# google/tfp-causalimpact

Hardware: AMD Instinct MI355X
Metric: posterior samples/sec (T=1000, 10 covariates) (higher is better)
Workload: dtype f32; 1 GPU; cfg2: T=1000, 10 covariates (P=11), LocalLinearTrend + spike-and-slab regression, Gibbs, W=112, S=1000; sampler=gibbs, chains_per_gpu=8, chains_total=8, parallelism=chains sharded over 1 GPU(s), no data-path collective, launcher=single process, collectives=none, ranks_seen=1

## Files before the change

tfp-causalimpact_amd/csrc/ci_api.hip:

```cpp
#include <hip/hip_runtime.h>

#include <algorithm>
#include <cerrno>
#include <cmath>
#include <cstdarg>
#include <cstdio>
#include <cstring>
#include <mutex>
#include <string>
#include <tuple>
#include <vector>

#include "../../include/causalimpact_amd.h"
#include "ci_kernels.h"
#include "ci_kernels8.h"
#define CI_SEASONAL_DECL_ONLY
#include "ci_seasonal.h"
#include "ci_wide.h"
#include "ci_seasonal_tp.h"
#include "ci_summary.h"
#include "ci_hmc.h"
#include "ci_score_seq.h"
#include "ci_gibbs64.h"
#include "ci_wide_score.h"
// ... 553 lines not shown
  if (pb->T < 3) return fail("T must be >= 3, got %d", pb->T);
  if (pb->P < 0 || pb->P > ci::MAXP_BIG)
    return fail("P must be in [0, %d], got %d", ci::MAXP_BIG, pb->P);
  if (pb->num_blocks < 0 || pb->num_blocks > CI_MAX_BLOCKS)
    return fail("num_blocks must be in [0, %d], got %d", CI_MAX_BLOCKS, pb->num_blocks);
  if (pb->num_blocks > 0) {
    int dfull = pb->has_slope ? 2 : 1;
    for (int k = 0; k < pb->num_blocks; ++k) {
      if (pb->num_seasons[k] < 2) return fail("num_seasons[%d] must be >= 2", k);
      dfull += pb->num_seasons[k];
    }
    if (use_wide(pb)) {
      if (wide_steps_per_thread(pb->T) > ci::WIDE_MAX_LC)
        return fail("T=%d exceeds the time-parallel seasonal path (max %d)", pb->T, ci::NT * ci::WIDE_MAX_LC);
    } else {
      if (dfull > ci::MW_MAXD)
        return fail("seasonal state too wide: %d > %d components (the limit of the multi-wavefront "
                    "seasonal kernel)", dfull, ci::MW_MAXD);
    }
  }
  if (pb->num_warmup < 0 || pb->num_results < 1) return fail("need num_warmup >= 0, num_results >= 1");
  if (pb->num_chains < 1 || pb->num_series < 1) return fail("need num_chains >= 1, num_series >= 1");
  if (pb->series_offset < 0 || pb->chain_offset < 0) return fail("series_offset and chain_offset must be >= 0");
  if (pb->num_blocks == 0 && steps_per_thread(pb->T) == 0 &&
      wide_steps_per_thread(pb->T) > ci::WIDE_MAX_LC)
    return fail("T=%d exceeds the longest supported series (%d)", pb->T, ci::NT * ci::WIDE_MAX_LC);
  return 0;
}

int ci_session_destroy(ci_session* s);

struct SessionGuard {
  ci_session* s;
  ~SessionGuard() { if (s) ci_session_destroy(s); }
};

static int validate_ragged(const ci_problem* pb, const int32_t* series_lengths) {
  if (validate(pb)) return 1;
  if (!series_lengths) return fail("series_lengths is NULL");
  if (pb->num_blocks > 0)
    return fail("ragged sessions hold trend models only: num_blocks must be 0, got %d", pb->num_blocks);
  if (pb->P > ci::MAXP)
    return fail("ragged sessions take at most %d design columns, got P=%d", ci::MAXP, pb->P);
  const int L = steps_per_thread(pb->T);
  if (L == 0)
    return fail("ragged sessions take series of at most %d steps, got T=%d", ci::NT * 16, pb->T);
  int longest = 0;
  for (int b = 0; b < pb->num_series; ++b) {
    const int tb = series_lengths[b];
    if (tb < 3) return fail("series_lengths[%d] must be >= 3, got %d", b, tb);
    if (tb > pb->T) return fail("series_lengths[%d] = %d exceeds the stride T=%d", b, tb, pb->T);
    if (tb > longest) longest = tb;
  }
  if (longest != pb->T)
    return fail("T must be the longest series of the session: max(series_lengths) = %d, T = %d",
                longest, pb->T);
  for (int b = 0; b < pb->num_series; ++b)
    if (steps_per_thread(series_lengths[b]) != L)
      return fail("series_lengths[%d] = %d runs %d steps per thread, the longest series (%d) runs %d: "
                  "all series of a ragged session must share that class",
                  b, series_lengths[b], steps_per_thread(series_lengths[b]), pb->T, L);
  return 0;
}

static int session_create_impl(const ci_problem* pb, const int32_t* series_lengths,
                               const int32_t* series_ids, const float* y, const uint8_t* mask,
                               const float* X, const uint8_t* season_change,
                               const ci_series_params* params, ci_session** out);

int ci_session_create(const ci_problem* pb, const float* y, const uint8_t* mask, const float* X,
                      const uint8_t* season_change, const ci_series_params* params,
                      ci_session** out) {
  if (validate(pb)) return 1;
  return session_create_impl(pb, nullptr, nullptr, y, mask, X, season_change, params, out);
}

int ci_session_create_ragged(const ci_problem* pb, const int32_t* series_lengths,
                             const int32_t* series_ids, const float* y, const uint8_t* mask,
                             const float* X, const ci_series_params* params, ci_session** out) {
  if (validate_ragged(pb, series_lengths)) return 1;
  if (series_ids)
    for (int b = 0; b < pb->num_series; ++b)
      if (series_ids[b] < 0) return fail("series_ids[%d] must be >= 0, got %d", b, series_ids[b]);
  return session_create_impl(pb, series_lengths, series_ids, y, mask, X, nullptr, params, out);
}

static int session_create_impl(const ci_problem* pb, const int32_t* series_lengths,
                               const int32_t* series_ids, const float* y, const uint8_t* mask,
                               const float* X, const uint8_t* season_change,
                               const ci_series_params* params, ci_session** out) {
  const bool ragged = series_lengths != nullptr;
  if (!y || !mask || !params || !out) return fail("NULL argument");
  if (pb->num_blocks > 0 && !season_change) return fail("season_change is NULL but num_blocks > 0");
  if (pb->P > 0 && !X) return fail("X is NULL but P=%d", pb->P);
  HIP_TRY(hipSetDevice(pb->device));
  ci_session* s = new ci_session();
  SessionGuard guard{s};
  s->pb = *pb;
  s->ragged = ragged;
  if (ragged) s->lengths.assign(series_lengths, series_lengths + pb->num_series);
  const ci_problem* caller_pb = pb;
  s->kpb = *pb;
  const bool bigp = pb->P > ci::MAXP;
  const bool long_trend = pb->num_blocks == 0 && ((steps_per_thread(pb->T) == 0 && !bigp) || wide_bigp_ok(pb));
  std::vector<uint8_t> no_changes;
  if (long_trend) {
    s->kpb.num_blocks = 1;
    s->kpb.num_seasons[0] = 2;
    s->kpb.flags &= ~CI_FLAG_SEQUENTIAL_SEASONAL;
    no_changes.assign((size_t)pb->T, 0);
    season_change = no_changes.data();
  }
  pb = &s->kpb;
  const int T = pb->T, P = pb->P, B = pb->num_series, C = pb->num_chains, S = pb->num_results;
  const int D = pb->has_slope ? 2 : 1;
  const int K = pb->num_blocks;
  (void)caller_pb;
  if (K == 0 && !bigp) {
    s->L = steps_per_thread(T);
    const ci::LdsLayout with_x = ci::make_layout(P, D, ci::NT * s->L, 1);
    s->x_in_lds = (P > 0 && with_x.total <= 150 * 1024) ? 1 : 0;
    s->lds_bytes = ci::make_layout(P, D, ci::NT * s->L, s->x_in_lds).total;
    const int pm = (P == 0) ? 0 : (P <= 16 ? (s->x_in_lds ? 1 : 3) : 2);
    s->fn = ragged ? pick_ragged_kernel(D, s->L, pm) : pick_kernel(D, s->L, pm);
    s->fn_prof = ragged ? nullptr : pick_kernel(D, s->L, pm + 8);
    if (!s->fn || (!ragged && !s->fn_prof)) return fail("no kernel for L=%d", s->L);
    char nm[96];
    snprintf(nm, sizeof(nm), ragged ? "ci::gibbs_kernel<%d,%d,%d,false,ragged>" : "ci::gibbs_kernel<%d,%d,%d,false>",
             D, s->L, pm);
    s->kernel_name = nm;
    int num_cus = 256;
    (void)hipDeviceGetAttribute(&num_cus, hipDeviceAttributeMultiprocessorCount, pb->device);
    const bool latency_regime = (long long)B * C <= (long long)num_cus;
    if ((pm == 1 || pm == 3) && latency_regime && !(pb->flags & CI_FLAG_FOUR_WAVES) && !ragged) {
      size_t base8 = 0;
      KernelFn f8 = pick_kernel8(D, s->L, 0, 0, &base8);
      size_t lds8 = base8 + (size_t)P * ci::NT * s->L * sizeof(float);
      int xg = 0;
      if (!f8 || lds8 > 160 * 1024) {
        f8 = pick_kernel8(D, s->L, 0, 1, &base8);
        lds8 = base8;
        xg = 1;
      }
      if (f8 && lds8 <= 160 * 1024) {
        s->fn = f8;
        s->fn_prof8 = xg ? nullptr : pick_kernel8(D, s->L, 1, 0, nullptr);
        if (s->fn_prof8)
          HIP_TRY(hipFuncSetAttribute((const void*)s->fn_prof8,
                                      hipFuncAttributeMaxDynamicSharedMemorySize, (int)lds8));
        s->eight_waves = true;
        if (const char* e_ = getenv("CI_SCHED_WORD")) {
          char* end_ = nullptr;
          const long v_ = strtol(e_, &end_, 0);
          if (end_ == e_ || *end_ != 0 || v_ < 0 || v_ > 0xFFFF)
            return fail("CI_SCHED_WORD must be an integer in [0, 65535], got '%s'", e_);
          s->sched_word = (int)v_;
        }
        s->lds_bytes = lds8;
        snprintf(nm, sizeof(nm), xg ? "ci::gibbs_kernel8<%d,%d,L2>" : "ci::gibbs_kernel8<%d,%d>", D, s->L);
        s->kernel_name = nm;
      }
    }
  } else {
    s->D_full = D;
    s->dred = D;
    for (int k = 0; k < K; ++k) { s->D_full += pb->num_seasons[k]; s->dred += pb->num_seasons[k] - 1; }
    s->wide = use_wide(pb);
    if (s->wide) {
      s->Lc = ci::wide_quad_steps(T);
      s->lds_bytes = ci::make_wlayout(P, s->dred).total;
      s->fn = (KernelFn)(bigp ? pick_wide_bigp_kernel(pb->has_slope, pb->num_seasons[0])
                              : pick_wide_kernel(pb->has_slope, pb->num_seasons[0]));
    } else {
      s->mw = s->D_full > 64 || (pb->flags & CI_FLAG_MULTIWAVE_SEASONAL) != 0;
      const int nwv = s->mw ? ci::MW_NWV : 1;
      const ci::SLayout in_lds = ci::make_slayout(T, P, K, s->D_full, s->dred, pb->has_slope, 0, nwv);
      s->seasonal_gws = in_lds.total > 150 * 1024 || (pb->flags & CI_FLAG_SEASONAL_WORKSPACE) != 0;
      const ci::SLayout lay = ci::make_slayout(T, P, K, s->D_full, s->dred, pb->has_slope,
                                               s->seasonal_gws ? 1 : 0, nwv);
      s->lds_bytes = lay.total;
      s->seasonal_ws_bytes = ((lay.t_total + 255) & ~(size_t)255) + (bigp ? ci::bigp_workspace_bytes(P) : 0);
    }
    const int tp_min_t = P > ci::MAXP ? 64 : 112;
    if (!s->wide && !s->mw && s->D_full <= ci::TP_MAXD && T >= tp_min_t && !(pb->flags & CI_FLAG_SEQUENTIAL_SEASONAL) &&
        !(pb->flags & CI_FLAG_SEASONAL_WORKSPACE)) {
      int num_cus = 256;
      (void)hipDeviceGetAttribute(&num_cus, hipDeviceAttributeMultiprocessorCount, pb->device);
      const long long groups = ((long long)B * C + 7) / 8 * 8;
      const ci::TpLds tl = ci::make_tplds(P, s->D_full);
      if (tl.total <= 160 * 1024) {
        int G = 1;
        while (G < ci::TP_MAXG && T / (2 * G * ci::TP_NWV) >= 16) G *= 2;
        int Gc = 1;
        if (!(pb->flags & CI_FLAG_NO_CLUSTER))
          while (Gc < G && groups * (2 * Gc) <= num_cus) Gc *= 2;
        s->tp = true;
        s->cluster = Gc;
        s->Lc = G;
        s->lds_bytes = tl.total;
        s->tp_ws_bytes = ci::make_tplayout(T, P, K, s->D_full, pb->has_slope, G).total;
        const int nq = ci::tp_nr(s->D_full) / 4;
        typedef void* (*TpFn)(void);
        static const TpFn tp_fns[9] = {nullptr, nullptr, ci_gibbs_seasonal_tp_fn_nq2, ci_gibbs_seasonal_tp_fn_nq3,
                                       ci_gibbs_seasonal_tp_fn_nq4, ci_gibbs_seasonal_tp_fn_nq5,
                                       ci_gibbs_seasonal_tp_fn_nq6, ci_gibbs_seasonal_tp_fn_nq7,
                                       ci_gibbs_seasonal_tp_fn_nq8};
        s->fn = (KernelFn)tp_fns[nq]();
      }
    }
    if (s->lds_bytes > 160 * 1024) {
      return fail("seasonal model needs %zu bytes of LDS per chain (max 163840): fewer covariates "
                  "or a narrower seasonal state", s->lds_bytes);
    }
    if (!s->wide && !s->tp) {
      const int which = (s->seasonal_gws ? 1 : 0) | (bigp ? 2 : 0);
      s->fn = (KernelFn)(s->mw ? ci_gibbs_seasonal_mw_fn(which) : ci_gibbs_seasonal_fn(which));
    }
    char nm[96];
    if (s->tp) snprintf(nm, sizeof(nm), "ci::gibbs_seasonal_tp_kernel<%d> %d chunks x%d", ci::tp_nr(s->D_full) / 4,
                        s->Lc * ci::TP_NWV, s->cluster);
    else if (s->wide) snprintf(nm, sizeof(nm), bigp ? "ci::gibbs_wide_kernel<%d,%d,bigp>" : "ci::gibbs_wide_kernel<%d,%d>", D, pb->num_seasons[0]);
    else if (s->mw) snprintf(nm, sizeof(nm), "ci::gibbs_seasonal_kernel<%s,%s,%d> (multi-wave)",
                             s->seasonal_gws ? "true" : "false", bigp ? "true" : "false", ci::MW_NWV);
    else snprintf(nm, sizeof(nm), "ci::gibbs_seasonal_kernel<%s,%s>", s->seasonal_gws ? "true" : "false",
                  bigp ? "true" : "false");
    s->kernel_name = nm;
  }
  HIP_TRY(hipFuncSetAttribute((const void*)s->fn, hipFuncAttributeMaxDynamicSharedMemorySize,
                              (int)s->lds_bytes));
  if (s->fn_prof) {
    const size_t lds_prof = K == 0 ? ci::make_layout(P, D, ci::NT * s->L, s->x_in_lds).total : s->lds_bytes;
    HIP_TRY(hipFuncSetAttribute((const void*)s->fn_prof, hipFuncAttributeMaxDynamicSharedMemorySize,
                                (int)lds_prof));
  }
  HIP_TRY(pool_stream_get(&s->stream));
  HIP_TRY(pool_event_get(&s->ev0));
  HIP_TRY(pool_event_get(&s->ev1));

  const size_t BT = (size_t)B * T, BCS = (size_t)B * C * S;
  HIP_TRY(s->y.alloc(BT));
  HIP_TRY(s->mask.alloc(BT));
  HIP_TRY(s->Xt.alloc((size_t)B * P * T));
  HIP_TRY(s->xtx.alloc((size_t)B * P * P));
  HIP_TRY(s->omega.alloc((size_t)B * P * P));
  HIP_TRY(s->wps.alloc(B));
  HIP_TRY(s->sp.alloc(B));
  HIP_TRY(s->o_obs.alloc(BCS));
  HIP_TRY(s->o_lscale.alloc(BCS));
  HIP_TRY(s->o_sscale.alloc(BCS));
  HIP_TRY(s->o_w.alloc(BCS * P));
  HIP_TRY(s->o_level.alloc(BCS * T));
  HIP_TRY(s->o_slope.alloc(pb->has_slope ? BCS * T : 0));
  HIP_TRY(s->o_pm.alloc((size_t)B * C * T));
  HIP_TRY(s->o_traj.alloc(BCS * T));
  if (ragged) {
    HIP_TRY(hipMemset(s->o_level.p, 0, s->o_level.n * sizeof(float)));
    if (s->o_slope.n) HIP_TRY(hipMemset(s->o_slope.p, 0, s->o_slope.n * sizeof(float)));
    HIP_TRY(hipMemset(s->o_pm.p, 0, s->o_pm.n * sizeof(float)));
    HIP_TRY(hipMemset(s->o_traj.p, 0, s->o_traj.n * sizeof(float)));
    HIP_TRY(s->series_T.alloc(B));
    HIP_TRY(hipMemcpy(s->series_T.p, series_lengths, B * sizeof(int), hipMemcpyHostToDevice));
    if (series_ids) {
      HIP_TRY(s->series_ids.alloc(B));
      HIP_TRY(hipMemcpy(s->series_ids.p, series_ids, B * sizeof(int), hipMemcpyHostToDevice));
    }
  }
  if (K > 0 || bigp) {
    HIP_TRY(s->season_change.alloc((size_t)K * T));
    HIP_TRY(s->ssp.alloc(B));
    HIP_TRY(s->p1_chol.alloc((size_t)B * s->dred * s->dred));
    s->inert_block = long_trend;
    if (!long_trend) {
      HIP_TRY(s->o_drift.alloc(BCS * K));
      HIP_TRY(s->o_seasonal.alloc(BCS * T * K));
    }
    if (s->wide) {
      HIP_TRY(s->ws.alloc((size_t)B * C * ci::wide_workspace_floats(s->dred, s->Lc)));
      int num_cus = 256;
      (void)hipDeviceGetAttribute(&num_cus, hipDeviceAttributeMultiprocessorCount, pb->device);
      const long long groups = ((long long)B * C + 7) / 8 * 8;
      s->cluster = 1;
      if (!(pb->flags & CI_FLAG_NO_CLUSTER) && P > 0 && (T & 3) == 0) {
        if (groups * 16 <= num_cus) s->cluster = 16;
        else if (groups * 8 <= num_cus) s->cluster = 8;
        else if (groups * 4 <= num_cus) s->cluster = 4;
        else if (groups * 2 <= num_cus) s->cluster = 2;
      }
      if ((s->cluster == 16 || s->cluster == 8) && getenv("CI_WIDE_DK_GLOBAL") == nullptr) {
        const size_t need = ci::make_wlayout(P, s->dred).big0 + ci::wide_dk_lds_bytes(s->Lc);
        if (need <= 160 * 1024 - 256) {
          s->dk_lds = 1;
          if (need > s->lds_bytes) {
            s->lds_bytes = need;
            HIP_TRY(hipFuncSetAttribute((const void*)s->fn, hipFuncAttributeMaxDynamicSharedMemorySize,
                                        (int)s->lds_bytes));
          }
        }
      }
      const size_t nseg = ((size_t)(T >> 2) + ci::NT - 1) / ci::NT;
      const size_t RS = (size_t)(P > 16 ? P : 16) + 4;
      HIP_TRY(s->csync.alloc((size_t)B * C * ci::CL_INTS));
      HIP_TRY(s->cpart.alloc((size_t)B * C * (nseg > 0 ? nseg : 1) * ci::NW * RS));
      HIP_TRY(s->cw.alloc((size_t)B * C * ci::wide_cw_floats(P)));
      HIP_TRY(s->cv.alloc((size_t)B * C * ci::wide_cv_doubles(P)));
    }
    else if (s->tp) {
      HIP_TRY(s->ws.alloc((size_t)B * C * (s->tp_ws_bytes / sizeof(float))));
      HIP_TRY(s->csync.alloc((size_t)B * C * ci::TPC_INTS));
// ... 1372 lines not shown
```

tfp-causalimpact_amd/csrc/ci_kernels8.h:

```cpp
#pragma once
#include "ci_kernels.h"

namespace ci {

constexpr int SCHED_DEFAULT = (2 << 4) | (1 << 6) | (0 << 8) | (2 << 10) | (2 << 12) | (0 << 14);
constexpr int NT8 = 512;
constexpr int NW8 = 8;
constexpr int PRE_MAXS = 16;

struct PreTables {
  double* tsw;
  double* V;
  double* rdk;
  double* hand;
};
constexpr size_t PRE_HALF_DOUBLES = PRE_MAXS * 16 + 16 * 16 + 16;
__host__ __device__ constexpr size_t pre_tables_bytes() {
  return sizeof(double) * (2 * PRE_HALF_DOUBLES + 20) + 16;
}
__device__ __forceinline__ PreTables pre_tables_at(unsigned char* base, int parity) {
  PreTables tb;
  double* d = (double*)base + (size_t)(parity & 1) * PRE_HALF_DOUBLES;
  tb.tsw = d; d += PRE_MAXS * 16;
  tb.V = d; d += 16 * 16;
  tb.rdk = d;
  tb.hand = (double*)base + 2 * PRE_HALF_DOUBLES;
  return tb;
}
constexpr int HAND_SCALE = 16, HAND_INTS = 17;

struct PreState {
  double c[4];
  double diag;
  double rdk;
  unsigned long long S;
  int n_sw;
  int valid;
};

template <int CTRL> __device__ __forceinline__ double dpp_ror_add_d(double v) {
  const int lo = __builtin_amdgcn_update_dpp(0, __double2loint(v), CTRL, 0xF, 0xF, false);
  const int hi = __builtin_amdgcn_update_dpp(0, __double2hiint(v), CTRL, 0xF, 0xF, false);
  return v + __hiloint2double(hi, lo);
}
__device__ __forceinline__ double row_sum16_d(double v) {
  v = dpp_ror_add_d<0x128>(v);
  v = dpp_ror_add_d<0x124>(v);
  v = dpp_ror_add_d<0x122>(v);
  v = dpp_ror_add_d<0x121>(v);
  return readlane_d(v, 0);
}

template <int KR>
__device__ __forceinline__ void sweep_rec_kr(QCols& m, int k, int lane, double& t_out, double& rd_out) {
  const int kq = k >> 2, j = lane & 15, q = lane >> 4;
  const double ckr = m.c[KR];
  const double rd = fast_rcp(readlane_d(ckr, k + 16 * kq));
  const double rowk = bperm_d(ckr, j + 16 * kq);
  const bool isk = j == k;
  const double t = isk ? 1.0 : rowk * rd;
  double colk[4];
#pragma unroll
  for (int r = 0; r < 4; ++r) colk[r] = bperm_d(m.c[r], k + 16 * q);
  __builtin_amdgcn_sched_barrier(0);
#pragma unroll
  for (int r = 0; r < 4; ++r) m.c[r] = isk ? colk[r] * rd : m.c[r] - colk[r] * t;
  m.c[KR] = (q == kq) ? (isk ? -rd : t) : m.c[KR];
  m.diag = isk ? -rd : m.diag - rowk * rowk * rd;
  t_out = t;
  rd_out = rd;
}
__device__ __forceinline__ void sweep_rec(QCols& m, int k, int lane, double& t_out, double& rd_out) {
  switch (k & 3) {
    case 0: sweep_rec_kr<0>(m, k, lane, t_out, rd_out); break;
    case 1: sweep_rec_kr<1>(m, k, lane, t_out, rd_out); break;
    case 2: sweep_rec_kr<2>(m, k, lane, t_out, rd_out); break;
    default: sweep_rec_kr<3>(m, k, lane, t_out, rd_out); break;
  }
}

struct PreRun {
  QCols m;
  double rdk;
  unsigned long long pending;
  int n;
  int phase;
};
__device__ __forceinline__ void pre_begin(PreRun& st, unsigned long long S) {
  st.pending = S;
  st.n = 0;
  st.rdk = 0.0;
  st.phase = 0;
}
__device__ __forceinline__ void pre_step(PreRun& st, const RegLds& R, int P, double var_next,
                                         unsigned long long S, int lane, const PreTables& tb,
                                         PreState& ps) {
  const int j = lane & 15, q = lane >> 4;
  const bool live = j < P;
  const int col = live ? j : 0;
  if (st.phase == 0) {
#pragma unroll
    for (int r = 0; r < 4; ++r) {
      const int i = 4 * q + r;
      double om = 0.0, xx = 0.0;
      if (live && i < P) {
        om = R.omega[i * P + col];
        xx = R.xtx[i * P + col];
      }
      st.m.c[r] = om * var_next + xx;
      st.m.p[r] = 0.0;
    }
    st.m.diag = live ? R.omega[col * P + col] * var_next + R.xtx[col * P + col] : 1.0;
    st.m.cb = 0.0; st.m.corner = 0.0; st.m.pdiag = 0.0;
    st.phase = st.pending != 0ull ? 1 : 2;
  } else if (st.phase == 1) {
    const int k = __builtin_amdgcn_readfirstlane(__ffsll((long long)st.pending) - 1);
    double t, rd;
    sweep_rec(st.m, k, lane, t, rd);
    if (q == 0) tb.tsw[st.n * 16 + j] = t;
    st.rdk = (j == k) ? rd : st.rdk;
    ++st.n;
    st.pending &= st.pending - 1ull;
    if (st.pending == 0ull) st.phase = 2;
  } else {
#pragma unroll
    for (int r = 0; r < 4; ++r) tb.V[(4 * q + r) * 16 + j] = st.m.c[r];
    if (q == 0) tb.rdk[j] = st.rdk;
    ps.n_sw = st.n;
#pragma unroll
    for (int r = 0; r < 4; ++r) ps.c[r] = st.m.c[r];
    ps.diag = st.m.diag;
    ps.rdk = st.rdk;
    ps.S = S;
    ps.valid = 1;
    st.phase = 3;
  }
}

__device__ __forceinline__ void weights_backsub(const PreTables& tb, const double* pre, int P,
                                                unsigned long long S, double mean, double new_scale,
                                                int lane, float* w) {
  const int j = lane & 15, q = lane >> 4;
  const bool live = j < P;
  const float zf = reinterpret_cast<const float*>(pre + 24)[live ? j : 0];
  const bool inS = ((S >> j) & 1ull) != 0ull;
  const int pos = __popcll(S & ((1ull << j) - 1ull));
  const int n_sw = __popcll(S);
  const double rsz = (double)__fsqrt_rn((float)tb.rdk[j]) * (double)zf;
  double tt[PRE_MAXS];
#pragma unroll
  for (int s = 0; s < PRE_MAXS; ++s) tt[s] = tb.tsw[s * 16 + j];
  double u = 0.0;
#pragma unroll
  for (int s = PRE_MAXS - 1; s >= 0; --s) {
    if (s < n_sw) {
      double dot = (inS && pos > s) ? tt[s] * u : 0.0;
      dot = dpp_ror_add_d<0x128>(dot);
      dot = dpp_ror_add_d<0x124>(dot);
      dot = dpp_ror_add_d<0x122>(dot);
      dot = dpp_ror_add_d<0x121>(dot);
      u = (inS && pos == s) ? rsz - dot : u;
    }
  }
  if (q == 0 && live) w[j] = inS ? (float)(mean + new_scale * u) : 0.f;
}

template <class PF, class Pub>
__device__ __forceinline__ double spike_slab_draw_pre(const RegLds& R, int P,
                                                      const DevSeriesParams& sp,
                                                      double prev_obs_scale, double g_obs,
                                                      int lane, PriorCarry& pc, const double* pre,
                                                      const PreTables& tb, const PreState& ps,
                                                      const float* red, PF& prof, Pub publish) {
  const double prev_var = prev_obs_scale * prev_obs_scale;
  const double a_post = sp.obs_conc + 0.5 * sp.n_obs;
  const bool all_in = sp.nonzero_prob >= 1.0;
  const int j = lane & 15, q = lane >> 4;
  const bool live = j < P;
  const int col = live ? j : 0;
  QCols m;
#pragma unroll
  for (int r = 0; r < 4; ++r) { m.c[r] = ps.c[r]; m.p[r] = pc.p[r]; }
  m.diag = ps.diag;
  m.pdiag = pc.pdiag;
  m.cb = live ? (double)red[col] : 0.0;
  m.corner = (double)red[RED_YTY];
  unsigned long long S = ps.S;
  {
    double v[16], bk[16];
#pragma unroll
    for (int g = 0; g < 4; ++g) {
      if (4 * g < P) {
#pragma unroll
        for (int k = 4 * g; k < 4 * g + 4; ++k) {
          v[k] = tb.V[k * 16 + j];
          bk[k] = (double)red[k];
        }
      } else {
#pragma unroll
        for (int k = 4 * g; k < 4 * g + 4; ++k) { v[k] = 0.0; bk[k] = 0.0; }
      }
    }
    double acc0 = 0.0, acc1 = 0.0;
#pragma unroll
    for (int k = 0; k < 16; k += 2) {
      acc0 = ((S >> k) & 1ull) ? fma(v[k], bk[k], acc0) : acc0;
      acc1 = ((S >> (k + 1)) & 1ull) ? fma(v[k + 1], bk[k + 1], acc1) : acc1;
    }
    const bool inj = ((S >> j) & 1ull) != 0ull;
    const double bj = m.cb;
    m.cb = live ? (inj ? 0.0 : bj) - (acc0 + acc1) : 0.0;
    m.corner -= row_sum16_d((live && inj) ? bj * m.cb : 0.0);
  }
  prof.tick(21);
  bool dirty = false;
  if (!all_in) {
    const int rank = reinterpret_cast<const int*>(pre + 16)[j];
    const double uflip = pre[j];
    const double logit_pi =
        (double)(__logf((float)sp.nonzero_prob) - __logf((float)(1.0 - sp.nonzero_prob)));
    int s_cur = 0;
    const double inv_prev_var = fast_rcp(prev_var);
    for (;;) {
      const bool in = ((S >> j) & 1ull) != 0ull;
      const double sg = in ? -1.0 : 1.0;
      const double rap = fast_rcp(sg * m.diag);
      const double beta_old = sp.obs_scale + 0.5 * m.corner;
      const double x = -0.5 * sg * m.cb * m.cb * rap * fast_rcp(beta_old);
      const double pscale = in ? inv_prev_var : prev_var;
      const double delta = 0.5 * (double)__logf((float)(sg * m.pdiag * pscale * rap)) +
                           sg * logit_pi - (a_post - 1.0) * fast_log1p(x);
      const float prob = 1.0f / (1.0f + __expf(-(float)delta));
      const bool acc = live && q == 0 && rank >= s_cur && uflip < (double)prob;
      unsigned long long cand = __ballot(acc);
      if (cand == 0ull) break;
      int best = -1, best_rank = 1 << 20;
      for (; cand != 0ull; cand &= cand - 1ull) {
        const int jj = __ffsll((long long)cand) - 1;
        const int rj = __builtin_amdgcn_readlane(rank, jj);
        if (rj < best_rank) { best_rank = rj; best = jj; }
      }
      best = __builtin_amdgcn_readfirstlane(best);
      sweep_q<true>(m, best, ((S >> best) & 1ull) != 0ull, lane);
      S ^= 1ull << best;
      s_cur = best_rank + 1;
      dirty = true;
    }
  }
  prof.tick(22);
#pragma unroll
  for (int r = 0; r < 4; ++r) pc.p[r] = m.p[r];
  pc.pdiag = m.pdiag;
  pc.S = S;
  pc.valid = 1;
  const double beta_post = sp.obs_scale + 0.5 * m.corner;
  double var = beta_post * fast_rcp(g_obs);
  if (var > sp.obs_ub) var = sp.obs_ub;
  const double new_scale = (double)__fsqrt_rn((float)var);
  const double mean = m.cb;
  if (publish(new_scale, mean, S, !dirty)) {
    prof.tick(23);
    return new_scale;
  }
  if (!dirty) {
    weights_backsub(tb, pre, P, S, mean, new_scale, lane, R.w);
  } else {
    const float zf = reinterpret_cast<const float*>(pre + 24)[col];
    double mu = 0.0, umine = 0.0;
    for (unsigned long long mm = S; mm != 0ull;) {
      const int aidx = __builtin_amdgcn_readfirstlane(63 - __clzll((long long)mm));
      mm &= ~(1ull << aidx);
      const double vaa = -readlane_d(m.diag, aidx);
      const double mua = readlane_d(mu, aidx);
      const double za = (double)__int_as_float(__builtin_amdgcn_readlane(__float_as_int(zf), aidx));
      const double ua = mua + (double)__fsqrt_rn((float)vaa) * za;
      const double t = unsweep_q(m, aidx, lane);
      if (j == aidx) umine = ua; else mu += t * (ua - mua);
    }
    if (q == 0 && live) R.w[j] = ((S >> j) & 1ull) ? (float)(mean + new_scale * umine) : 0.f;
  }
  wave_sync();
  prof.tick(23);
  return new_scale;
}


template <int D, int L> struct Lay8 {
  static constexpr size_t TP = (size_t)NT * L;
  static constexpr size_t a16(size_t x) { return (x + 15) & ~(size_t)15; }
  static constexpr size_t off_ctx = 0;
  static constexpr size_t off_xtx = a16(sizeof(SerialCtx));
  static constexpr size_t off_omega = off_xtx + 16 * 16 * sizeof(double);
  static constexpr size_t off_bvec = off_omega + 16 * 16 * sizeof(double);
  static constexpr size_t off_w = off_bvec + a16(20 * sizeof(double));
  static constexpr size_t off_scal = off_w + 16 * sizeof(float);
  static constexpr size_t off_red = off_scal + 32 * sizeof(float);
  static constexpr size_t off_slots = off_red + 32 * sizeof(float);
  static constexpr size_t off_xlast = off_slots + 3 * NW * 16 * sizeof(float);
  static constexpr size_t off_gam = off_xlast + a16((size_t)NT * D * sizeof(float));
  static constexpr size_t off_pre = off_gam + a16((8 + 64 + 4) * sizeof(double));
  static constexpr size_t off_tgv = off_pre + a16(pre_tables_bytes());
  static constexpr size_t off_z = off_tgv + TP * sizeof(float);
  static constexpr bool PARK = L >= 8;
  static constexpr size_t off_xw = off_z + 3 * TP * sizeof(float);
  static constexpr size_t off_y = off_xw + (PARK ? TP * sizeof(float) : 0);
  static constexpr size_t off_x = off_y + (PARK ? TP * sizeof(float) : 0);
  static __host__ __device__ constexpr size_t total(int P) { return off_x + (size_t)P * TP * sizeof(float); }
};
enum Scal8 { SC8_INIT_LOC = 8, SC8_INIT_VAR = 9, SC8_INIT_SVAR = 10, SC8_ZINIT = 12 };

template <int D, int L, bool PROF = false, bool XG = false>
__global__ __launch_bounds__(NT8) void gibbs_kernel8(KArgs a) {
  using PF = typename std::conditional<PROF, Prof, NoProf>::type;
  using LY = Lay8<D, L>;
  extern __shared__ __attribute__((aligned(16))) unsigned char smem[];
  const int tid = threadIdx.x, lane = tid & 63;
  const int wave = __builtin_amdgcn_readfirstlane(tid >> 6);
  const int series = blockIdx.x / a.C, chain = blockIdx.x % a.C;
  const int T = a.T, P = a.P;
  constexpr int TPAD = NT * L;
  SerialCtx* cx = (SerialCtx*)(smem + LY::off_ctx);
  float* scal = (float*)(smem + LY::off_scal);
  float* red = (float*)(smem + LY::off_red);
  float* slots = (float*)(smem + LY::off_slots);
  float* xlast = (float*)(smem + LY::off_xlast);
  float* wls = (float*)(smem + LY::off_w);
  float* tgv = (float*)(smem + LY::off_tgv);
  float* zb = (float*)(smem + LY::off_z);
  float* xwb = (float*)(smem + LY::off_xw);
  float* ybuf = (float*)(smem + LY::off_y);
  double* gam = (double*)(smem + LY::off_gam);
  const size_t chain_lin = (size_t)series * a.C + chain;
  const int n_iter = a.W + a.S;

  Rng rng;
  rng.k0 = stream_key0(a.seed0, a.series_stream_base, series);
  rng.k1 = stream_key1(a.seed1, a.series_stream_base, series);
  rng.chain = (uint32_t)(a.chain_offset + chain);

  const float* yg = a.y + (size_t)series * T;
  const uint8_t* mg = a.mask + (size_t)series * T;
  const float* Xg = a.Xt + (size_t)series * P * T;
  const float* Xs = XG ? Xg : (const float*)(smem + LY::off_x);
  const bool xwide = L % 4 == 0 && (T & 3) == 0 && (reinterpret_cast<uintptr_t>(Xg) & 15) == 0;
  RegLds R;
  R.xtx = (double*)(smem + LY::off_xtx);
  R.omega = (double*)(smem + LY::off_omega);
  R.aug[0] = R.aug[1] = R.pri[0] = R.pri[1] = R.chol = R.zv = R.uperm = nullptr;
  R.nz = R.perm = R.idx = nullptr;
  R.bvec = (double*)(smem + LY::off_bvec);
  R.w = wls;
  if (tid == 0) {
    cx->sp = a.sp[series];
    cx->obs_scale = cx->sp.obs_scale0;
    cx->level_scale = cx->sp.level_scale0;
    cx->slope_scale = cx->sp.slope_scale0;
    cx->R = R;
    cx->scal = scal;
    cx->red = red;
    cx->out_obs = a.out_obs;
    cx->out_level_scale = a.out_level_scale;
    cx->out_slope_scale = a.out_slope_scale;
    cx->out_weights = a.out_weights;
    cx->chain_lin = chain_lin;
    cx->rng = rng;
    cx->P = P; cx->T = T; cx->D = D; cx->W = a.W; cx->S = a.S; cx->n_iter = n_iter;
    cx->prof = nullptr;
    scal[SC_OBS_DK] = (float)cx->sp.obs_scale0;
    scal[SC8_INIT_LOC] = (float)cx->sp.init_level_loc;
    scal[SC8_INIT_VAR] = (float)(cx->sp.init_level_scale * cx->sp.init_level_scale);
    scal[SC8_INIT_SVAR] = (float)(cx->sp.init_slope_scale * cx->sp.init_slope_scale);
  }
  {
    for (int e = tid; e < P * P; e += NT8) {
      R.xtx[e] = a.xtx[(size_t)series * P * P + e];
      R.omega[e] = a.omega[(size_t)series * P * P + e];
    }
    if constexpr (!XG) {
      float* xw_ = (float*)(smem + LY::off_x);
      for (int j = 0; j < P; ++j)
        for (int t = tid; t < TPAD; t += NT8) xw_[j * TPAD + t] = (t < T) ? Xg[(size_t)j * T + t] : 0.f;
    }
    if (tid < 16) wls[tid] = 0.f;
  }
  __syncthreads();
  unsigned char* pre_base = smem + LY::off_pre;

  if (wave > NW) {
    const int e = wave - NW - 1;
    constexpr int NTASK = (D == 2) ? 3 : 2;
    constexpr int ROUNDS = NTASK * L;
    constexpr int N0 = ROUNDS / 3, N1 = (ROUNDS - N0) / 2;
    const int k_lo = e == 0 ? 0 : (e == 1 ? N0 : N0 + N1);
    const int k_hi = e == 0 ? N0 : (e == 1 ? N0 + N1 : ROUNDS);
    const int n_my = k_hi - k_lo;
    PF eprof;
    eprof.start(a.prof, a.prof != nullptr && blockIdx.x == 0 && wave == NW + 1 && lane == 0);
    auto normals_round = [&](int k, uint32_t it_for) __attribute__((always_inline)) {
      const int task = k / L, blk = k - task * L;
      const int slot = (D == 2) ? task : (task == 0 ? 0 : 2);
      const uint32_t site = slot == 0 ? SITE_PRIOR_LEVEL : (slot == 1 ? SITE_PRIOR_SLOPE : SITE_PRIOR_OBS);
      const int c = 64 * blk + lane;
      const U4 r = site_call(rng, it_for, site, 0, (uint32_t)c);
      float z[4];
      normals4(r, z);
      *reinterpret_cast<float4*>(zb + (size_t)slot * TPAD + 4 * c) = make_float4(z[0], z[1], z[2], z[3]);
    };
    auto role_work = [&](int it_next) __attribute__((always_inline)) {
      if (it_next > n_iter) return;
      if (e == 0) {
        serial_gammas<1>(cx, it_next, lane, gam + 4 * (it_next & 1));
      } else if (e == 1) {
        if (it_next < n_iter) spike_slab_randoms(rng, (uint32_t)it_next, P, lane, gam + 8 + 32 * (it_next & 1));
      } else if (it_next < n_iter) {
        float zi[1];
        fill_normals<1>(rng, (uint32_t)it_next, SITE_PRIOR_INIT, 0, (uint32_t)lane, zi);
        asm volatile("" : "+v"(zi[0]));
        if (lane < D) scal[SC8_ZINIT + 2 * (it_next & 1) + lane] = zi[0];
      }
    };
    role_work(0);
    for (int k = k_lo; k < k_hi; ++k) normals_round(k, 0u);
    eprof.tick(30);
    const int sched = (a.dbg & 0xFFFF) ? (a.dbg & 0xFFFF) : SCHED_DEFAULT;
    const int mode = sched & 3;
    const int scale = L >= 4 ? L / 4 : 1;
    const int c_3 = e == 2 ? 0 : ((sched >> 10) & 3) * scale, c_4 = ((sched >> 12) & 3) * scale,
              c_a = ((sched >> 14) & 3) * scale;
    const int r_3 = mode == 1 ? n_my : (mode == 2 ? 0 : (c_3 < n_my ? c_3 : n_my));
    const int r_4 = mode == 1 ? n_my : (mode == 2 ? 0 : (r_3 + c_4 < n_my ? r_3 + c_4 : n_my));
    const int r_5 = mode == 2 ? 0 : (n_my - c_a > r_4 ? n_my - c_a : r_4);
    for (int it = 0; it <= n_iter; ++it) {
      __syncthreads();
      eprof.tick(31);
      xt_sums_wave<L, 2, XG>(tgv, Xs, TPAD, P, 2 * wave, wave == NW8 - 1, red, lane, T, xwide);
      eprof.tick(30);
      __syncthreads();
      eprof.tick(31);
      role_work(it + 1);
      eprof.tick(30);
      __syncthreads();
      eprof.tick(31);
      if (e == 2 && it < n_iter) {
        const PreTables tb = pre_tables_at(pre_base, it);
        const int* hi_ = reinterpret_cast<const int*>(tb.hand + HAND_INTS);
        if (hi_[2] != 0) {
          const unsigned long long S = ((unsigned long long)(unsigned)hi_[1] << 32) | (unsigned)hi_[0];
          weights_backsub(tb, gam + 8 + 32 * (it & 1), P, S, tb.hand[lane & 15], tb.hand[HAND_SCALE],
                          lane, wls);
        }
      }
      int r = 0;
      if (it < n_iter)
        for (; r < r_3; ++r) normals_round(k_lo + r, (uint32_t)(it + 1));
      eprof.tick(30);
      __syncthreads();
      eprof.tick(31);
      if (it == n_iter) break;
      for (; r < r_4; ++r) normals_round(k_lo + r, (uint32_t)(it + 1));
      eprof.tick(30);
      __syncthreads();
      eprof.tick(31);
      for (; r < r_5; ++r) normals_round(k_lo + r, (uint32_t)(it + 1));
      eprof.tick(30);
      __syncthreads();
      eprof.tick(31);
      for (; r < n_my; ++r) normals_round(k_lo + r, (uint32_t)(it + 1));
      eprof.tick(30);
    }
    return;
  }

  if (wave == NW) {
    PriorCarry pc;
    pc.valid = 0; pc.S = 0ull; pc.pdiag = 0.0;
#pragma unroll
    for (int r = 0; r < 4; ++r) pc.p[r] = 0.0;
    PreState ps;
    ps.valid = 0; ps.S = 0ull; ps.n_sw = 0; ps.diag = 1.0; ps.rdk = 0.0;
#pragma unroll
    for (int r = 0; r < 4; ++r) ps.c[r] = 0.0;
    PF rprof;
    rprof.start(a.prof, a.prof != nullptr && blockIdx.x == 0 && lane == 0);
    double obs_scale = cx->sp.obs_scale0, level_scale = cx->sp.level_scale0, slope_scale = cx->sp.slope_scale0;
    const DevSeriesParams sp = cx->sp;
    float* o_obs = a.out_obs;
    float* o_ls = a.out_level_scale;
    float* o_ss = a.out_slope_scale;
    float* o_w = a.out_weights;
    const int sched = (a.dbg & 0xFFFF) ? (a.dbg & 0xFFFF) : SCHED_DEFAULT;
    const int mode = sched & 3;
    for (int it = 0; it <= n_iter; ++it) {
      __syncthreads();
      __builtin_amdgcn_s_setprio(3);
      xt_sums_wave<L, 2, XG>(tgv, Xs, TPAD, P, 2 * wave, false, red, lane, T, xwide);
      __syncthreads();
      rprof.tick(16);
      const PreTables tb = pre_tables_at(pre_base, it);
      if (lane < P + 1) R.bvec[lane] = (double)red[lane < P ? lane : RED_YTY];
      const float wprev = lane < P ? wls[lane] : 0.f;
      const double* gm = gam + 4 * (it & 1);
      const double g_level = gm[0], g_slope = gm[1], g_obs = gm[2];
      const double emit_obs = obs_scale;
      rprof.tick(20);
      auto publish4 = [&](double ns, double mean, unsigned long long S, bool clean) __attribute__((always_inline)) {
        if (lane == 0) scal[SC_OBS_DK] = (float)ns;
        if (lane < 16) tb.hand[lane] = mean;
        if (lane == 0) {
          tb.hand[HAND_SCALE] = ns;
          int* hi_ = reinterpret_cast<int*>(tb.hand + HAND_INTS);
          hi_[0] = (int)(unsigned)(S & 0xFFFFFFFFull);
          hi_[1] = (int)(unsigned)(S >> 32);
          hi_[2] = clean ? 1 : 0;
        }
        rprof.tick(22);
        __builtin_amdgcn_s_setprio(0);
        __syncthreads();
        rprof.tick(18);
        return clean;
      };
      auto publish1 = [&](double ns) __attribute__((always_inline)) { (void)publish4(ns, 0.0, 0ull, false); };
      if (it < n_iter) {
        if (ps.valid && ps.S == pc.S) {
          obs_scale = spike_slab_draw_pre(R, P, sp, obs_scale, g_obs, lane, pc, gam + 8 + 32 * (it & 1), tb,
                                          ps, red, rprof, publish4);
        } else {
          NoProf np;
          wave_sync();
          obs_scale = spike_slab_draw_regs(R, P, sp, obs_scale, g_obs, rng, (uint32_t)it, lane, np, pc,
                                           gam + 8 + 32 * (it & 1), publish1);
        }
      } else {
        publish1(obs_scale);
      }
      rprof.tick(23);
      auto after_b3 = [&]() __attribute__((always_inline)) {
        if (it > 0) {
          auto clipped_scale = [](double scale, double ss, double g, double ub) {
            const double s = (double)__fsqrt_rn((float)((scale + 0.5 * ss) * fast_rcp(g)));
            return s < ub ? s : ub;
          };
          double ssl = 0.0, sss = 0.0;
#pragma unroll
          for (int w = 0; w < NW; ++w) {
            ssl += (double)red[RED_INC + 2 * w];
            sss += (double)red[RED_INC + 2 * w + 1];
          }
          level_scale = clipped_scale(sp.level_scale, ssl, g_level, sp.level_ub);
          if (D == 2) slope_scale = clipped_scale(sp.slope_scale, sss, g_slope, sp.slope_ub);
          const int s = it - 1 - a.W;
          if (s >= 0) {
            const size_t o = chain_lin * a.S + s;
            if (lane == 0) {
              if (o_obs) o_obs[o] = (float)emit_obs;
              if (o_ls) o_ls[o] = (float)level_scale;
              if (o_ss) o_ss[o] = (float)(D == 2 ? slope_scale : 0.0);
            }
            if (o_w && lane < P) o_w[o * P + lane] = wprev;
          }
        }
      };
      if (it == n_iter) {
        __syncthreads();
        after_b3();
        break;
      }
      const PreTables tbn = pre_tables_at(pre_base, it + 1);
      const double var_next = obs_scale * obs_scale;
      PreRun st;
      pre_begin(st, pc.S);
      const int n_sw = __popcll(pc.S);
      const int p_3 = (sched >> 4) & 3, p_4 = (sched >> 6) & 3, p_a = (sched >> 8) & 3;
      const int s_3 = mode == 1 ? n_sw + 2 : (mode == 2 ? 0 : 1 + (p_3 < n_sw ? p_3 : n_sw));
      const int s_4 = mode == 1 ? n_sw + 2 : (mode == 2 ? 0 : (s_3 + p_4 < 1 + n_sw ? s_3 + p_4 : 1 + n_sw));
      const int s_5 = mode == 1 ? n_sw + 2 : (mode == 2 ? 0 : (1 + n_sw - p_a > s_4 ? 1 + n_sw - p_a : s_4));
      int step = 0;
      for (; st.phase != 3 && step < s_3; ++step) pre_step(st, R, P, var_next, pc.S, lane, tbn, ps);
      rprof.tick(19);
      __syncthreads();
      rprof.tick(17);
      after_b3();
      for (; st.phase != 3 && step < s_4; ++step) pre_step(st, R, P, var_next, pc.S, lane, tbn, ps);
      rprof.tick(19);
      __syncthreads();
      rprof.tick(29);
      for (; st.phase != 3 && step < s_5; ++step) pre_step(st, R, P, var_next, pc.S, lane, tbn, ps);
      rprof.tick(19);
      __syncthreads();
      rprof.tick(29);
      for (; st.phase != 3; ++step) pre_step(st, R, P, var_next, pc.S, lane, tbn, ps);
      rprof.tick(19);
    }
    return;
  }

  __builtin_amdgcn_s_setprio(1);
  const int t0 = tid * L;
  float yv[L];
  uint32_t maskbits = 0;
#pragma unroll
  for (int l = 0; l < L; ++l) {
    const int t = t0 + l;
    const bool in = t < T;
    yv[l] = in ? yg[t] : 0.f;
    const bool m = in ? (mg[t] != 0) : true;
    if (m) { maskbits |= (1u << l); yv[l] = 0.f; }
  }
  if constexpr (LY::PARK) store_targets<L>(ybuf, t0, yv);
  const float init_loc = scal[SC8_INIT_LOC], init_var = scal[SC8_INIT_VAR], init_svar = scal[SC8_INIT_SVAR];
  const DevSeriesParams* spp = &cx->sp;
  const double sp_level_scale0 = spp->level_scale0, sp_slope_scale0 = spp->slope_scale0;
  const double sp_level_scale = spp->level_scale, sp_slope_scale = spp->slope_scale;
  const double sp_level_ub = spp->level_ub, sp_slope_ub = spp->slope_ub;
  float lev[L], slp[L], xw[L], pm_acc[L];
#pragma unroll
  for (int l = 0; l < L; ++l) { lev[l] = 0.f; slp[l] = 0.f; xw[l] = 0.f; pm_acc[l] = 0.f; }
  float* o_level = a.out_level ? a.out_level + chain_lin * a.S * T : nullptr;
  float* o_slope = a.out_slope ? a.out_slope + chain_lin * a.S * T : nullptr;
  float* o_traj = a.out_traj ? a.out_traj + chain_lin * a.S * T : nullptr;
  PF prof;
  prof.start(a.prof, a.prof != nullptr && blockIdx.x == 0 && tid == 0);
  for (int it = 0; it <= n_iter; ++it) {
    {
      float tg[L], yq[L];
      if constexpr (LY::PARK) {
        lds_row_load<L>(ybuf + t0, yq);
      } else {
#pragma unroll
        for (int l = 0; l < L; ++l) yq[l] = yv[l];
      }
#pragma unroll
      for (int l = 0; l < L; ++l) {
        const bool obs = ((maskbits >> l) & 1u) == 0u;
        tg[l] = obs ? (yq[l] - lev[l]) : 0.f;
      }
      store_targets<L>(tgv, t0, tg);
      xlast[tid * D] = lev[L - 1];
      if constexpr (D == 2) xlast[tid * D + 1] = slp[L - 1];
    }
    __syncthreads();
    xt_sums_wave<L, 2, XG>(tgv, Xs, TPAD, P, 2 * wave, false, red, lane, T, xwide);
    {
      float ssl = 0.f, sss = 0.f;
      float pl = (tid > 0) ? xlast[(tid - 1) * D] : 0.f;
      float ps_ = 0.f;
      if constexpr (D == 2) ps_ = (tid > 0) ? xlast[(tid - 1) * D + 1] : 0.f;
#pragma unroll
      for (int l = 0; l < L; ++l) {
        const int t = t0 + l;
        if (t >= 1 && t < T) {
          float dl = lev[l] - pl;
          if constexpr (D == 2) {
            dl -= ps_;
            const float ds = slp[l] - ps_;
            sss = fmaf(ds, ds, sss);
          }
          ssl = fmaf(dl, dl, ssl);
        }
        pl = lev[l];
        if constexpr (D == 2) ps_ = slp[l];
      }
      const float s1 = wave_prefix_dpp(ssl), s2 = wave_prefix_dpp(sss);
      if (lane == 63) {
        red[RED_INC + 2 * wave] = s1;
        red[RED_INC + 2 * wave + 1] = s2;
      }
    }
    const float so_prev = scal[SC_OBS_DK];
    __syncthreads();
    prof.tick(0);

    float zl[L], zs[L], zo[L];
    const float* zit = zb + t0;
    lds_row_load<L>(zit, zl);
    if constexpr (D == 2) {
      lds_row_load<L>(zit + TPAD, zs);
    } else {
#pragma unroll
      for (int l = 0; l < L; ++l) zs[l] = 0.f;
    }
    lds_row_load<L>(zit + 2 * TPAD, zo);
    if (it > a.W) {
      const int s = it - 1 - a.W;
      float zp[L];
      fill_normals<L>(rng, (uint32_t)(it - 1), SITE_PRED, 0, (uint32_t)t0, zp);
      float tr[L];
      if constexpr (LY::PARK) {
        float xwp[L], acc[L];
        lds_row_load<L>(xwb + t0, xwp);
        float* pm = a.out_pred_mean ? a.out_pred_mean + chain_lin * T : nullptr;
        const bool vec = (T & 3) == 0;
        if (pm != nullptr && s > 0) {
          if (vec) {
#pragma unroll
            for (int q = 0; q < L / 4; ++q) {
              const int t = t0 + 4 * q;
              const float4 v = t < T ? *(const float4*)(pm + t) : make_float4(0.f, 0.f, 0.f, 0.f);
              acc[4 * q] = v.x; acc[4 * q + 1] = v.y; acc[4 * q + 2] = v.z; acc[4 * q + 3] = v.w;
            }
          } else {
#pragma unroll
            for (int l = 0; l < L; ++l) acc[l] = t0 + l < T ? pm[t0 + l] : 0.f;
          }
        } else {
#pragma unroll
          for (int l = 0; l < L; ++l) acc[l] = 0.f;
        }
#pragma unroll
        for (int l = 0; l < L; ++l) {
          const float loc = lev[l] + xwp[l];
          acc[l] += loc;
          tr[l] = fmaf(so_prev, zp[l], loc);
        }
        if (pm != nullptr) {
          if (vec) {
#pragma unroll
            for (int q = 0; q < L / 4; ++q) {
              const int t = t0 + 4 * q;
              if (t < T) *(float4*)(pm + t) = make_float4(acc[4 * q], acc[4 * q + 1], acc[4 * q + 2], acc[4 * q + 3]);
            }
          } else {
#pragma unroll
            for (int l = 0; l < L; ++l)
              if (t0 + l < T) pm[t0 + l] = acc[l];
          }
        }
      } else {
#pragma unroll
        for (int l = 0; l < L; ++l) {
          const float loc = lev[l] + xw[l];
          pm_acc[l] += loc;
          tr[l] = fmaf(so_prev, zp[l], loc);
        }
      }
      const size_t row = (size_t)s * T;
      bool vec_done = false;
      if constexpr (L % 4 == 0) {
        if ((T & 3) == 0) {
          vec_done = true;
#pragma unroll
          for (int q = 0; q < L / 4; ++q) {
            const int t = t0 + 4 * q;
            if (t < T) {
              if (o_level) *(float4*)(o_level + row + t) = make_float4(lev[4 * q], lev[4 * q + 1], lev[4 * q + 2], lev[4 * q + 3]);
              if (o_slope) *(float4*)(o_slope + row + t) = make_float4(slp[4 * q], slp[4 * q + 1], slp[4 * q + 2], slp[4 * q + 3]);
              if (o_traj) *(float4*)(o_traj + row + t) = make_float4(tr[4 * q], tr[4 * q + 1], tr[4 * q + 2], tr[4 * q + 3]);
            }
          }
        }
      }
      if (!vec_done) {
#pragma unroll
        for (int l = 0; l < L; ++l) {
          const int t = t0 + l;
          if (t < T) {
            if (o_level) o_level[row + t] = lev[l];
            if (o_slope) o_slope[row + t] = slp[l];
            if (o_traj) o_traj[row + t] = tr[l];
          }
        }
      }
    }
    Vec<D> sig;
    PElem<D> pincl = pelem_identity<D>();
    {
      auto clipped_scale = [](double scale, double ss, double g, double ub) {
        const double s = (double)__fsqrt_rn((float)((scale + 0.5 * ss) * fast_rcp(g)));
        return s < ub ? s : ub;
      };
      double level_scale = sp_level_scale0, slope_scale = sp_slope_scale0;
      if (it > 0) {
        const double* gm = gam + 4 * (it & 1);
        double ssl = 0.0, sss = 0.0;
#pragma unroll
        for (int w = 0; w < NW; ++w) {
          ssl += (double)red[RED_INC + 2 * w];
          sss += (double)red[RED_INC + 2 * w + 1];
        }
        level_scale = clipped_scale(sp_level_scale, ssl, gm[0], sp_level_ub);
        if constexpr (D == 2) slope_scale = clipped_scale(sp_slope_scale, sss, gm[1], sp_slope_ub);
      }
      sig.v[0] = (float)level_scale;
      if constexpr (D == 2) sig.v[1] = (float)slope_scale;
      if (it < n_iter) pincl = dk_prior_begin<D, L>(sig, zl, zs, slots, lane, wave);
    }
    const bool publish = a.progress != nullptr && it > a.W &&
                         ((it - a.W) % a.progress_every == 0 || it - a.W == a.S);
    if (publish) asm volatile("s_waitcnt vmcnt(0)" ::: "memory");
    prof.tick(2);
    __syncthreads();
    prof.tick(1);
    if (publish) {
      if (tid == 0) {
        __builtin_amdgcn_fence(__ATOMIC_RELEASE, "");
        asm volatile("s_waitcnt vmcnt(0)" ::: "memory");
        __hip_atomic_store(a.progress + chain_lin, (unsigned int)(it - a.W), __ATOMIC_RELAXED,
                           __HIP_MEMORY_SCOPE_SYSTEM);
      }
    }
    if (it == n_iter) {
      __syncthreads();
      break;
    }

    DkModel<D> md;
    {
      const float so = scal[SC_OBS_DK];
      md.H = so * so;
      md.sig = sig;
      md.a1 = vzero<D>();
      md.a1.v[0] = init_loc;
      md.p1.v[0] = init_var;
      if constexpr (D == 2) md.p1.v[1] = init_svar;
    }
    Vec<D> q;
#pragma unroll
    for (int i = 0; i < D; ++i) q.v[i] = md.sig.v[i] * md.sig.v[i];
    const PElem<D> ppre = dk_prior_finish<D>(pincl, slots, lane, wave);
    const FMElem<D> fme = dk_matrix_chunk<D, L>(md, q, maskbits, tid);
    const FMElem<D> mincl = dk_matrix_scan_begin<D>(fme, slots + NW * 16, lane, wave);
    prof.tick(24);
    __syncthreads();
    float Pin[D * (D + 1) / 2];
    dk_matrix_scan_finish<D>(mincl, slots + NW * 16, lane, wave, Pin);
    DkMats<D, L> km;
    dk_matrix_local<D, L>(md, q, maskbits, tid, Pin, km);
// ... 102 lines not shown
```

Before: 1.168 million posterior samples/sec.

## Double-buffer prior normals in LDS so RNG waves can run an iteration ahead

For small L (L<=4), the prior-normal buffer in LDS becomes two buffers selected by iteration parity. The extra RNG waves get a new segment-based schedule that fills the next iteration's normals during the current one, with a configurable lookahead packed into the upper bits of the schedule word. The consumer side reads the buffer matching the current iteration. The aim is to hide random-number generation behind the main sampler work, at the cost of more LDS and a more complex barrier schedule.

```diff
diff --git a/tfp-causalimpact_amd/csrc/ci_api.hip b/tfp-causalimpact_amd/csrc/ci_api.hip
--- a/tfp-causalimpact_amd/csrc/ci_api.hip
+++ b/tfp-causalimpact_amd/csrc/ci_api.hip
@@ -729,8 +729,8 @@
         if (const char* e_ = getenv("CI_SCHED_WORD")) {
           char* end_ = nullptr;
           const long v_ = strtol(e_, &end_, 0);
-          if (end_ == e_ || *end_ != 0 || v_ < 0 || v_ > 0xFFFF)
-            return fail("CI_SCHED_WORD must be an integer in [0, 65535], got '%s'", e_);
+          if (end_ == e_ || *end_ != 0 || v_ < 0 || v_ > ci::SCHED_WORD_MAX)
+            return fail("CI_SCHED_WORD must be an integer in [0, %d], got '%s'", ci::SCHED_WORD_MAX, e_);
           s->sched_word = (int)v_;
         }
         s->lds_bytes = lds8;
diff --git a/tfp-causalimpact_amd/csrc/ci_kernels8.h b/tfp-causalimpact_amd/csrc/ci_kernels8.h
--- a/tfp-causalimpact_amd/csrc/ci_kernels8.h
+++ b/tfp-causalimpact_amd/csrc/ci_kernels8.h
@@ -4,6 +4,8 @@
 namespace ci {
 
 constexpr int SCHED_DEFAULT = (2 << 4) | (1 << 6) | (0 << 8) | (2 << 10) | (2 << 12) | (0 << 14);
+constexpr int SCHED_WORD_MAX = (1 << 25) - 1;
+template <int L> constexpr int sched_lookahead_default() { return 0; }
 constexpr int NT8 = 512;
 constexpr int NW8 = 8;
 constexpr int PRE_MAXS = 16;
@@ -301,8 +303,9 @@
   static constexpr size_t off_pre = off_gam + a16((8 + 64 + 4) * sizeof(double));
   static constexpr size_t off_tgv = off_pre + a16(pre_tables_bytes());
   static constexpr size_t off_z = off_tgv + TP * sizeof(float);
+  static constexpr int ZBUFS = L <= 4 ? 2 : 1;
   static constexpr bool PARK = L >= 8;
-  static constexpr size_t off_xw = off_z + 3 * TP * sizeof(float);
+  static constexpr size_t off_xw = off_z + ZBUFS * 3 * TP * sizeof(float);
   static constexpr size_t off_y = off_xw + (PARK ? TP * sizeof(float) : 0);
   static constexpr size_t off_x = off_y + (PARK ? TP * sizeof(float) : 0);
   static __host__ __device__ constexpr size_t total(int P) { return off_x + (size_t)P * TP * sizeof(float); }
@@ -404,7 +407,9 @@
       const U4 r = site_call(rng, it_for, site, 0, (uint32_t)c);
       float z[4];
       normals4(r, z);
-      *reinterpret_cast<float4*>(zb + (size_t)slot * TPAD + 4 * c) = make_float4(z[0], z[1], z[2], z[3]);
+      float* zw = zb + (size_t)slot * TPAD + 4 * c;
+      if constexpr (LY::ZBUFS == 2) zw += (it_for & 1u) * (3 * TPAD);
+      *reinterpret_cast<float4*>(zw) = make_float4(z[0], z[1], z[2], z[3]);
     };
     auto role_work = [&](int it_next) __attribute__((always_inline)) {
       if (it_next > n_iter) return;
@@ -419,6 +424,61 @@
         if (lane < D) scal[SC8_ZINIT + 2 * (it_next & 1) + lane] = zi[0];
       }
     };
+    if constexpr (LY::ZBUFS == 2) {
+      const int sched = (a.dbg & 0xFFFF) ? (a.dbg & 0xFFFF) : SCHED_DEFAULT;
+      const int la = a.dbg != 0 ? (a.dbg >> 16) & 0x1FF : sched_lookahead_default<L>();
+      const int mode = sched & 3;
+      const int scale = L >= 4 ? L / 4 : 1;
+      auto cap = [&](int x) { return x < n_my ? x : n_my; };
+      const int c_3 = e == 2 ? 0 : ((sched >> 10) & 3) * scale, c_4 = ((sched >> 12) & 3) * scale,
+                c_a = ((sched >> 14) & 3) * scale;
+      const int q_2 = cap((la & 7) * scale), q_s = cap(q_2 + ((la >> 3) & 7) * scale);
+      const int lead = cap(((la >> 6) & 7) * scale);
+      const int f_3 = mode == 1 ? n_my : (mode == 2 ? q_s : cap(q_s + c_3));
+      const int f_4 = mode == 1 ? n_my : (mode == 2 ? q_s : cap(f_3 + c_4));
+      const int f_5 = mode == 2 ? q_s : (n_my - c_a > f_4 ? n_my - c_a : f_4);
+      const int t_2 = cap(q_2 + lead), t_s = cap(q_s + lead), t_3 = f_3 + lead, t_4 = f_4 + lead,
+                t_5 = f_5 + lead;
+      role_work(0);
+      int cj = 0, cr = 0;
+      for (int it = 0; it <= n_iter; ++it) {
+#pragma unroll 1
+        for (int seg = 0; seg < 6; ++seg) {
+          if (seg == 1) {
+            xt_sums_wave<L, 2, XG>(tgv, Xs, TPAD, P, 2 * wave, wave == NW8 - 1, red, lane, T, xwide);
+          } else {
+            if (seg == 2) role_work(it + 1);
+            if (seg == 3 && e == 2 && it < n_iter) {
+              const PreTables tb = pre_tables_at(pre_base, it);
+              const int* hi_ = reinterpret_cast<const int*>(tb.hand + HAND_INTS);
+              if (hi_[2] != 0) {
+                const unsigned long long S = ((unsigned long long)(unsigned)hi_[1] << 32) | (unsigned)hi_[0];
+                weights_backsub(tb, gam + 8 + 32 * (it & 1), P, S, tb.hand[lane & 15], tb.hand[HAND_SCALE],
+                                lane, wls);
+              }
+            }
+            int tj = it + 1;
+            int tr = seg == 0 ? t_2 : (seg == 2 ? t_s : (seg == 3 ? t_3 : (seg == 4 ? t_4 : t_5)));
+            if (tr > n_my) { tr -= n_my; ++tj; }
+            if (tj > n_iter) { tj = n_iter; tr = n_my; }
+            while (cj < tj || (cj == tj && cr < tr)) {
+              if (cr < n_my) {
+                normals_round(k_lo + cr, (uint32_t)cj);
+                ++cr;
+              } else {
+                ++cj;
+                cr = 0;
+              }
+            }
+          }
+          eprof.tick(seg < 3 ? 15 : 30);
+          __syncthreads();
+          eprof.tick(31);
+          if (seg == 3 && it == n_iter) return;
+        }
+      }
+      return;
+    }
     role_work(0);
     for (int k = k_lo; k < k_hi; ++k) normals_round(k, 0u);
     eprof.tick(30);
@@ -671,7 +731,7 @@
     prof.tick(0);
 
     float zl[L], zs[L], zo[L];
-    const float* zit = zb + t0;
+    const float* zit = zb + t0 + (LY::ZBUFS == 2 ? (it & 1) * (3 * TPAD) : 0);
     lds_row_load<L>(zit, zl);
     if constexpr (D == 2) {
       lds_row_load<L>(zit + TPAD, zs);
```

New measurement: 990,800 posterior samples/sec. 0.848x the previous value.
